# aleju/face-generator

Hardware: AMD Instinct MI355X
Metric: GAN train images/sec (G+D step) at 32x32x3 bs128 (higher is better)
Workload: dtype f32

## Files before the change

### face_generator_amd/csrc/thin.hip

```cpp
#include "fg_internal.h"
#ifdef FG_MEASURE
#define FG_THIN_DBG_BIT(v, b) ((v) & (b))
#else
#define FG_THIN_DBG_BIT(v, b) 0
#endif
#include <string.h>
#include <stdlib.h>
typedef float tw_f32x16 __attribute__((ext_vector_type(16)));
typedef float tw_f32x4 __attribute__((ext_vector_type(4)));

__device__ __forceinline__ float wave_sum_x(float v) {
#pragma unroll
    for (int o = 32; o > 0; o >>= 1) v += __shfl_xor(v, o, 64);
    return v;
}

template <int K, int CS, int CJ>
__global__ __launch_bounds__(256) void thin_in_kernel(const float* __restrict__ in, const float* __restrict__ Wp,
                                                      const float* __restrict__ bias, float* __restrict__ out, int B,
                                                      int H, int W, int flip, int Cw) {
    constexpr int PAD = (K - 1) / 2;
    const int lane = threadIdx.x & 63;
    const int wave = __builtin_amdgcn_readfirstlane(threadIdx.x >> 6);
    const int cb = blockIdx.y * (CJ * 64) + lane;
    float w[K * K * CS][CJ];
#pragma unroll
    for (int t = 0; t < K * K * CS; ++t)
#pragma unroll
        for (int j = 0; j < CJ; ++j) w[t][j] = Wp[(size_t)t * Cw + cb + 64 * j];
    float bv[CJ];
#pragma unroll
    for (int j = 0; j < CJ; ++j) bv[j] = bias ? bias[cb + 64 * j] : 0.f;
    const int npix = B * H * W;
    const int nwaves = gridDim.x * 4;
    for (int pix0 = blockIdx.x * 4 + wave; pix0 < npix; pix0 += 2 * nwaves) {
        float v[2][K * K * CS];
#pragma unroll
        for (int u = 0; u < 2; ++u) {
            const int pix = min(pix0 + u * nwaves, npix - 1);
            const int x = pix % W;
            const int t = pix / W;
            const int y = t % H;
            const int b = t / H;
#pragma unroll
            for (int dy = 0; dy < K; ++dy) {
                const int yy = y + (flip ? PAD - dy : dy - PAD);
                const int yc = min(max(yy, 0), H - 1);
#pragma unroll
                for (int dx = 0; dx < K; ++dx) {
                    const int xx = x + (flip ? PAD - dx : dx - PAD);
                    const int xc = min(max(xx, 0), W - 1);
                    const bool ok = yy == yc && xx == xc;
                    const float* ip = in + ((size_t)(b * H + yc) * W + xc) * CS;
#pragma unroll
                    for (int s = 0; s < CS; ++s) {
                        const float tv = ip[s];
                        v[u][(dy * K + dx) * CS + s] = ok ? tv : 0.f;
                    }
                }
            }
        }
#pragma unroll
        for (int u = 0; u < 2; ++u) {
            const int pix = pix0 + u * nwaves;
            if (pix >= npix) break;
            float acc[CJ];
#pragma unroll
            for (int j = 0; j < CJ; ++j) acc[j] = bv[j];
#pragma unroll
            for (int t = 0; t < K * K * CS; ++t)
#pragma unroll
                for (int j = 0; j < CJ; ++j) acc[j] = fmaf(v[u][t], w[t][j], acc[j]);
#pragma unroll
            for (int j = 0; j < CJ; ++j) out[(size_t)pix * Cw + cb + 64 * j] = acc[j];
        }
    }
}

template <int CS, int CJ>
__global__ __launch_bounds__(256) void thin_in_row3_kernel(const float* __restrict__ in, const float* __restrict__ Wp,
                                                           const float* __restrict__ bias, float* __restrict__ out,
                                                           int B, int H, int W, int flip, int Cw) {
    const int lane = threadIdx.x & 63;
    const int wave = __builtin_amdgcn_readfirstlane(threadIdx.x >> 6);
    const int cb = blockIdx.y * (CJ * 64) + lane;
    float w[9 * CS][CJ];
#pragma unroll
    for (int t = 0; t < 9; ++t)
#pragma unroll
        for (int s = 0; s < CS; ++s)
#pragma unroll
            for (int j = 0; j < CJ; ++j) w[t * CS + s][j] = Wp[(size_t)((flip ? 8 - t : t) * CS + s) * Cw + cb + 64 * j];
    float bv[CJ];
#pragma unroll
    for (int j = 0; j < CJ; ++j) bv[j] = bias ? bias[cb + 64 * j] : 0.f;
    const int row = blockIdx.x * 4 + wave;
    if (row >= B * H) return;
    const int y = row % H;
    const float* rp[3];
    bool rok[3];
#pragma unroll
    for (int dy = 0; dy < 3; ++dy) {
        const int yy = y + dy - 1;
        rok[dy] = (unsigned)yy < (unsigned)H;
        rp[dy] = in + (size_t)(row + (rok[dy] ? dy - 1 : 0)) * W * CS;
    }
    float win[3][3][CS];
#define FG_LOADCOL(slot, xc)                                                                        \
    {                                                                                               \
        const bool cok = (unsigned)(xc) < (unsigned)W;                                              \
        const int xcl = cok ? (xc) : 0;                                                             \
        _Pragma("unroll") for (int dy = 0; dy < 3; ++dy)                                            \
            _Pragma("unroll") for (int s = 0; s < CS; ++s) {                                        \
                const float tv = rp[dy][xcl * CS + s];                                              \
                win[slot][dy][s] = (cok && rok[dy]) ? tv : 0.f;                                     \
            }                                                                                       \
    }
    FG_LOADCOL(2, -1)
    FG_LOADCOL(0, 0)
    float* orow = out + (size_t)row * W * Cw + cb;
    for (int x0 = 0; x0 < W; x0 += 3) {
#pragma unroll
        for (int u = 0; u < 3; ++u) {
            const int x = x0 + u;
            if (x >= W) break;
            FG_LOADCOL((u + 1) % 3, x + 1)
            float acc[CJ];
#pragma unroll
            for (int j = 0; j < CJ; ++j) acc[j] = bv[j];
#pragma unroll
            for (int dy = 0; dy < 3; ++dy)
#pragma unroll
                for (int dx = 0; dx < 3; ++dx)
#pragma unroll
                    for (int s = 0; s < CS; ++s)
#pragma unroll
                        for (int j = 0; j < CJ; ++j)
                            acc[j] = fmaf(win[(u + dx + 2) % 3][dy][s], w[(dy * 3 + dx) * CS + s][j], acc[j]);
#pragma unroll
            for (int j = 0; j < CJ; ++j) orow[(size_t)x * Cw + 64 * j] = acc[j];
        }
    }
#undef FG_LOADCOL
}

template <int K, int CS>
__global__ __launch_bounds__(256) void thin_in_rows_kernel(const float* __restrict__ in, const float* __restrict__ Wp,
                                                           const float* __restrict__ bias, float* __restrict__ out,
                                                           int B, int H, int W, int flip, int Cw) {
    constexpr int PAD = (K - 1) / 2;
    constexpr int TR = 4, NPX = 4;
    constexpr int SEG = (NPX + K - 1) * CS;
    constexpr int SEG4 = (SEG + 3) / 4 * 4;
    extern __shared__ __attribute__((aligned(16))) float tile[];
    const int WP = (W + 2 * PAD + 3) / 4 * 4 + 4;
    const int lane = threadIdx.x & 63, wave = threadIdx.x >> 6;
    const int c = blockIdx.y * 64 + lane;
    float w[K * K * CS];
#pragma unroll
    for (int t = 0; t < K * K; ++t)
#pragma unroll
        for (int s = 0; s < CS; ++s) w[t * CS + s] = Wp[(size_t)((flip ? K * K - 1 - t : t) * CS + s) * Cw + c];
    const float bv = bias ? bias[c] : 0.f;
    const int strips_per_img = (H + TR - 1) / TR;
    const int b = blockIdx.x / strips_per_img, y0 = (blockIdx.x - b * strips_per_img) * TR;
    for (int i = threadIdx.x; i < (TR + 2 * PAD) * WP * CS; i += 256) {
        const int s = i % CS;
        const int t = i / CS;
        const int xx = t % WP - PAD, yy = y0 + t / WP - PAD;
        float v = 0.f;
        if ((unsigned)yy < (unsigned)H && (unsigned)xx < (unsigned)W) v = in[((size_t)(b * H + yy) * W + xx) * CS + s];
        tile[i] = v;
    }
    __syncthreads();
    const int rows = min(TR, H - y0);
    const int gpr = (W + NPX - 1) / NPX;
    for (int grp = wave; grp < rows * gpr; grp += 4) {
        const int r = grp / gpr, x0 = (grp - r * gpr) * NPX;
        float acc[NPX];
#pragma unroll
        for (int q = 0; q < NPX; ++q) acc[q] = bv;
#pragma unroll
        for (int dy = 0; dy < K; ++dy) {
            float seg[SEG4];
            const float* sp = tile + ((r + dy) * WP + x0) * CS;
#pragma unroll
            for (int i = 0; i < SEG4; ++i) seg[i] = sp[i];
#pragma unroll
            for (int dx = 0; dx < K; ++dx)
#pragma unroll
                for (int s = 0; s < CS; ++s)
#pragma unroll
                    for (int q = 0; q < NPX; ++q) acc[q] = fmaf(seg[(q + dx) * CS + s], w[(dy * K + dx) * CS + s], acc[q]);
            __builtin_amdgcn_sched_barrier(0);
        }
#pragma unroll
        for (int q = 0; q < NPX; ++q)
            if (x0 + q < W) out[((size_t)(b * H + y0 + r) * W + x0 + q) * Cw + c] = acc[q];
    }
}

__global__ __launch_bounds__(256) void thin_in_generic_kernel(const float* __restrict__ in, const float* __restrict__ Wp,
                                                              const float* __restrict__ bias, float* __restrict__ out,
                                                              int B, int H, int W, int Cs, int Cw, int K, int flip,
                                                              int cblk) {
    const int PAD = (K - 1) / 2;
    const int pl = threadIdx.x / cblk, tc = threadIdx.x - pl * cblk;
    const int PL = 256 / cblk;
    const int c = blockIdx.y * cblk + tc;
    const float bv = bias ? bias[c] : 0.f;
    const int npix = B * H * W;
    const int p0 = blockIdx.x * 128;
    for (int j = pl; j < 128; j += PL) {
        const int pix = p0 + j;
        if (pix >= npix) break;
        const int x = pix % W;
        const int t = pix / W;
        const int y = t % H;
        const int b = t / H;
        float acc = bv;
        for (int dy = 0; dy < K; ++dy) {
            const int yy = y + (flip ? PAD - dy : dy - PAD);
            if ((unsigned)yy >= (unsigned)H) continue;
            for (int dx = 0; dx < K; ++dx) {
                const int xx = x + (flip ? PAD - dx : dx - PAD);
                if ((unsigned)xx >= (unsigned)W) continue;
                const float* ip = in + ((size_t)(b * H + yy) * W + xx) * Cs;
                for (int s = 0; s < Cs; ++s) acc = fmaf(ip[s], Wp[(size_t)((dy * K + dx) * Cs + s) * Cw + c], acc);
            }
        }
        out[(size_t)pix * Cw + c] = acc;
    }
}

struct ThinEpi { const float* slope; float* y; const float* x; float* part; };
template <int EPI>
__device__ __forceinline__ void thin_epi_store(const ThinEpi& e, float sl, float* __restrict__ out, size_t idx, float v0, float v1,
                                               float x0, float x1, float& s) {
    if constexpr (EPI == 2) {
        s = fmaf(x0 > 0.f ? 0.f : x0, v0, s);
        s = fmaf(x1 > 0.f ? 0.f : x1, v1, s);
        out[idx] = x0 > 0.f ? v0 : sl * v0;
        out[idx + 32] = x1 > 0.f ? v1 : sl * v1;
    } else {
        out[idx] = v0;
        out[idx + 32] = v1;
        if constexpr (EPI == 1) {
            e.y[idx] = v0 > 0.f ? v0 : sl * v0;
            e.y[idx + 32] = v1 > 0.f ? v1 : sl * v1;
        }
    }
}
template <int EPI>
__device__ __forceinline__ void thin_epi_prefetch(const ThinEpi& e, int tile, int h, int npix, int Cw, int cbj, float (&x0)[16],
                                                  float (&x1)[16]) {
    if constexpr (EPI == 2) {
#pragma unroll
        for (int r = 0; r < 16; ++r) {
            const int p = tile * 32 + (r & 3) + 8 * (r >> 2) + 4 * h;
            const size_t idx = (size_t)(p < npix ? p : 0) * Cw + cbj;
            x0[r] = e.x[idx];
            x1[r] = e.x[idx + 32];
        }
    }
}
__device__ __forceinline__ void thin_epi_finish(const ThinEpi& e, float s, int lane, int wave) {
    if (!e.part) return;
#pragma unroll
    for (int o = 32; o > 0; o >>= 1) s += __shfl_xor(s, o, 64);
    if (lane == 0) e.part[((size_t)blockIdx.y * gridDim.x + blockIdx.x) * 4 + wave] = s;
}

template <int CS, int EPI>
__global__ __launch_bounds__(256) void thin_in_mfma_kernel(const float* __restrict__ in, const float* __restrict__ Wp,
                                                           const float* __restrict__ bias, float* __restrict__ out,
                                                           int npix, int H, int W, int flip, int Cw, int lgH, int lgW,
                                                           const ThinEpi epi, int nt_store) {
    constexpr int NA = 9 * CS;
    constexpr int KS = (NA + 1) / 2;
    constexpr int TS_LD = 68;
    __shared__ __attribute__((aligned(16))) float tsm[EPI == 0 ? 4 : 1][EPI == 0 ? 32 * TS_LD : 4];
    const int lane = threadIdx.x & 63, wave = threadIdx.x >> 6;
    const int cb = blockIdx.y * 64;
    const int h = lane >> 5, j = lane & 31;
    float wb[KS][2];
    int kdesc[KS];
#pragma unroll
    for (int ks = 0; ks < KS; ++ks) {
        const int k = 2 * ks + h;
        const bool valid = k < NA;
        const int tap = valid ? k / CS : 0, sc = valid ? k - tap * CS : 0;
        const size_t widx = (size_t)((flip ? 8 - tap : tap) * CS + sc) * Cw + cb + j;
        wb[ks][0] = valid ? Wp[widx] : 0.f;
        wb[ks][1] = valid ? Wp[widx + 32] : 0.f;
        kdesc[ks] = (tap / 3) | ((tap % 3) << 2) | (sc << 4) | ((valid ? 1 : 0) << 8);
    }
    const float b0 = bias ? bias[cb + j] : 0.f, b1 = bias ? bias[cb + 32 + j] : 0.f;
    const bool p2 = lgW >= 0 && lgH >= 0;
    const int ntiles = (npix + 31) / 32;
    const float esl = EPI ? epi.slope[0] : 1.f;
    float es = 0.f;
    auto load_a = [&](int tile, float (&av)[KS]) {
        const int pix = tile * 32 + j;
        const bool ok = pix < npix;
        int x, y, t;
        if (p2) { x = pix & (W - 1); t = pix >> lgW; y = t & (H - 1); }
        else { t = pix / W; x = pix - t * W; y = t % H; }
#pragma unroll
        for (int ks = 0; ks < KS; ++ks) {
            const int d = kdesc[ks];
            const int yy = y + (d & 3) - 1, xx = x + ((d >> 2) & 3) - 1;
            float a = 0.f;
// ... 841 lines not shown
            }                                                                                                        \
            hipLaunchKernelGGL((thin_out_rows_mfma_kernel<KK, CC>), grid, dim3(256), lds, ctx->stream, in, Wp, rbuf, B, H, W, Cw); \
            FG_CHECK_LAUNCH(ctx);                                                                                    \
            hipLaunchKernelGGL((thin_out_rows_gather_kernel<KK, CC>), dim3(fg_cdiv(npix * CC, 256)), dim3(256), 0,    \
                               ctx->stream, rbuf, bias, out, npix, W, sigmoid);                                      \
            FG_CHECK_LAUNCH(ctx);                                                                                    \
            return FG_OK;                                                                                            \
        }
        TOR(5, 1) TOR(5, 3) TOR(7, 1) TOR(7, 3)
#undef TOR
    }
    dim3 grid(fg_cdiv(npix, 64));
    const long long in_bytes = (long long)npix * Cw * 4;
    {
        const bool use_slab = (ctx->fusion & FG_FUSE_THIN_SLAB) != 0;
        int R = 0;
        if (W >= 4 && W <= 128) {
            const int rmax = (80 * 1024 / (29 * 4)) / W - 2;
            int rt = (int)(((long long)H * B + 255) / 256);
            if (rt > rmax) rt = rmax;
            if (rt > H) rt = H;
            if (rt < 2) rt = 2;
            for (int pass = 0; pass < 2 && !R; ++pass)
                for (int r = rt; r >= 2; --r)
                    if (((r + 2) * W) % 32 == 0 && (pass == 1 || H % r == 0)) { R = r; break; }
            if (!R && rmax >= 2)
                for (int r = rt + 1; r <= rmax; ++r) if (((r + 2) * W) % 32 == 0) { R = r; break; }
        }
        if (use_slab && in_bytes < (long long)FG_OOB_T && k == 3 && R >= 2 && (Cw == 64 || Cw == 128) && Cs <= 3 &&
            ((R + 2) * W) % 32 == 0) {
            const int nblk = B * ((H + R - 1) / R);
            const size_t lds = (size_t)(R + 2) * W * 29 * sizeof(float);
#define TOS(JJ, CC)                                                                                                  \
            if (Cw == JJ * 64 && Cs == CC) {                                                                         \
                static bool attr = false;                                                                            \
                if (!attr) {                                                                                         \
                    FG_HIP(ctx, hipFuncSetAttribute((const void*)thin_out_slab_mfma_kernel<JJ, CC>,                  \
                                                    hipFuncAttributeMaxDynamicSharedMemorySize, 160 * 1024));        \
                    attr = true;                                                                                     \
                }                                                                                                    \
                hipLaunchKernelGGL((thin_out_slab_mfma_kernel<JJ, CC>), dim3(nblk), dim3(256), lds, ctx->stream, in, Wp, bias, \
                                   out, H, W, R, flip, sigmoid, (int)in_bytes);                                      \
                FG_CHECK_LAUNCH(ctx);                                                                                \
                return FG_OK;                                                                                        \
            }
            TOS(1, 1) TOS(1, 3) TOS(2, 1) TOS(2, 3)
#undef TOS
        }
    }
    if (in_bytes < (long long)FG_OOB_T && k == 3 && W % 4 == 0) {
        int nblk = fg_cdiv(fg_cdiv(npix, 4), 4);
        if (nblk > 4096) nblk = 4096;
#define TOW(JJ, CC)                                                                                                  \
        if (Cw == JJ * 64 && Cs == CC) {                                                                             \
            hipLaunchKernelGGL((thin_out_win_kernel<JJ, CC>), dim3(nblk), dim3(256), 0, ctx->stream, in, Wp, bias, out, B, H, \
                               W, flip, sigmoid, (int)in_bytes);                                                     \
            FG_CHECK_LAUNCH(ctx);                                                                                    \
            return FG_OK;                                                                                            \
        }
        TOW(1, 1) TOW(1, 3) TOW(2, 1) TOW(2, 3)
#undef TOW
    }
    if (in_bytes < (long long)FG_OOB_T) {
        int nblk = fg_cdiv(fg_cdiv(npix, 4), 4);
        if (nblk > 4096) nblk = 4096;
#define TO(KK, JJ, CC)                                                                                              \
    if (k == KK && Cw == JJ * 64 && Cs == CC) {                                                                     \
        hipLaunchKernelGGL((thin_out_kernel<KK, JJ, CC, 4>), dim3(nblk), dim3(256), 0, ctx->stream, in, Wp, bias, out, B, \
                           H, W, flip, sigmoid, (int)in_bytes);                                                     \
        FG_CHECK_LAUNCH(ctx);                                                                                       \
        return FG_OK;                                                                                               \
    }
        TO(3, 1, 1) TO(3, 1, 3) TO(3, 2, 1) TO(3, 2, 3)
    }
#undef TO
    if (Cw % 32 == 0 && (k == 3 || k == 5 || k == 7) && (Cs == 1 || Cs == 3)) {
        const int tp = 16 + k - 1;
        const size_t lds = (size_t)tp * tp * 36 * sizeof(float);
        dim3 tgrid(B * ((H + 15) / 16) * ((W + 15) / 16));
#define TOT(KK, CC)                                                                                                  \
    if (k == KK && Cs == CC) {                                                                                       \
        static bool attr = false;                                                                                    \
        if (!attr) {                                                                                                 \
            FG_HIP(ctx, hipFuncSetAttribute((const void*)thin_out_tiled_kernel<KK, CC>,                              \
                                            hipFuncAttributeMaxDynamicSharedMemorySize, (int)lds));                  \
            attr = true;                                                                                             \
        }                                                                                                            \
        hipLaunchKernelGGL((thin_out_tiled_kernel<KK, CC>), tgrid, dim3(256), lds, ctx->stream, in, Wp, bias, out, B, H, \
                           W, Cw, flip, sigmoid);                                                                    \
        FG_CHECK_LAUNCH(ctx);                                                                                        \
        return FG_OK;                                                                                                \
    }
        TOT(3, 1) TOT(3, 3) TOT(5, 1) TOT(5, 3) TOT(7, 1) TOT(7, 3)
#undef TOT
    }
    hipLaunchKernelGGL(thin_out_generic_kernel, grid, dim3(256), 0, ctx->stream, in, Wp, bias, out, B, H, W, Cw, Cs, k,
                       flip, sigmoid);
    FG_CHECK_LAUNCH(ctx);
    return FG_OK;
}

#define TW_BLOCKS FG_THIN_WGRAD_BLOCKS
#define TW_ROWS 4
template <int K, int CS>
__global__ __launch_bounds__(256) void thin_wgrad_kernel(const float* __restrict__ thin, const float* __restrict__ wide,
                                                         float* __restrict__ part, int B, int H, int W, int Cw, int sgn,
                                                         int cblk) {
    constexpr int PAD = (K - 1) / 2;
    constexpr int NA = K * K * CS;
    extern __shared__ float sh[];
    const int WP = W + 2 * PAD;
    float* tile = sh;
    float* red = sh + (TW_ROWS + 2 * PAD) * WP * CS;
    const int pl = threadIdx.x / cblk, tc = threadIdx.x - pl * cblk;
    const int PL = 256 / cblk;
    const int c = blockIdx.y * cblk + tc;
    const int strips_per_img = (H + TW_ROWS - 1) / TW_ROWS;
    const int nstrips = B * strips_per_img;
    float acc[NA];
#pragma unroll
    for (int t = 0; t < NA; ++t) acc[t] = 0.f;
    for (int st = blockIdx.x; st < nstrips; st += gridDim.x) {
        const int b = st / strips_per_img, y0 = (st - b * strips_per_img) * TW_ROWS;
        __syncthreads();
        for (int i = threadIdx.x; i < (TW_ROWS + 2 * PAD) * WP * CS; i += 256) {
            const int s = i % CS;
            const int t = i / CS;
            const int xx = t % WP - PAD, yy = y0 + t / WP - PAD;
            float v = 0.f;
            if ((unsigned)yy < (unsigned)H && (unsigned)xx < (unsigned)W) v = thin[((size_t)(b * H + yy) * W + xx) * CS + s];
            tile[i] = v;
        }
        __syncthreads();
        const int rows = min(TW_ROWS, H - y0);
        const int npx = rows * W;
        for (int j0 = pl; j0 < npx; j0 += 4 * PL) {
            float wv[4];
#pragma unroll
            for (int u = 0; u < 4; ++u) {
                const int j = j0 + u * PL;
                wv[u] = j < npx ? wide[((size_t)(b * H + y0) * W + j) * Cw + c] : 0.f;
            }
#pragma unroll
            for (int u = 0; u < 4; ++u) {
                const int j = j0 + u * PL;
                if (j >= npx) break;
                const int ry = j / W, rx = j - ry * W;
#pragma unroll
                for (int dy = 0; dy < K; ++dy)
#pragma unroll
                    for (int dx = 0; dx < K; ++dx) {
                        const float* tp = tile + ((ry + PAD + sgn * (dy - PAD)) * WP + rx + PAD + sgn * (dx - PAD)) * CS;
#pragma unroll
                        for (int s = 0; s < CS; ++s)
                            acc[(dy * K + dx) * CS + s] = fmaf(tp[s], wv[u], acc[(dy * K + dx) * CS + s]);
                    }
            }
        }
    }
    float* dst = part + (size_t)blockIdx.x * NA * Cw;
    if (PL == 1) {
#pragma unroll
        for (int t = 0; t < NA; ++t) dst[(size_t)t * Cw + c] = acc[t];
    } else {
        __syncthreads();
#pragma unroll
        for (int t = 0; t < NA; ++t) red[(pl * NA + t) * cblk + tc] = acc[t];
        __syncthreads();
        if (pl == 0) {
#pragma unroll
            for (int t = 0; t < NA; ++t) {
                float s = 0.f;
                for (int q = 0; q < PL; ++q) s += red[(q * NA + t) * cblk + tc];
                dst[(size_t)t * Cw + c] = s;
            }
        }
    }
}

template <int K, int CS, int PADDED = 0, int ONES = 0>
__global__ __launch_bounds__(256) void thin_wgrad_mfma_kernel(const float* __restrict__ thin, const float* __restrict__ wide,
                                                              float* __restrict__ part, int B, int H, int W, int Cw, int sgn, int lgH, int lgW) {
    constexpr int PAD = (K - 1) / 2;
    constexpr int NA = K * K * CS;
    constexpr int NCT = (NA + 31) / 32;
    static_assert(NA % 32 != 0, "the ones column needs an idle column");
    constexpr int CTO = NA / 32;
    __shared__ float red[4][2][16][64];
    const int lane = threadIdx.x & 63, wave = threadIdx.x >> 6;
    const int cbase = blockIdx.y * 64;
    const long long npix = (long long)B * H * W, npairs = (npix + 1) / 2;
    const int j = lane & 31, k = lane >> 5;
    const bool ones_lane = ONES && (CTO * 32 + j == NA);
    constexpr int NR = NA + ONES;
    int oy[NCT], ox[NCT], sch[NCT];
    bool jok[NCT];
#pragma unroll
    for (int ct = 0; ct < NCT; ++ct) {
        const int jj = ct * 32 + j;
        jok[ct] = jj < NA;
        const int tap = jok[ct] ? jj / CS : 0;
        sch[ct] = jok[ct] ? jj - tap * CS : 0;
        oy[ct] = sgn * (tap / K - PAD); ox[ct] = sgn * (tap % K - PAD);
    }
    const int Wp = W + 2 * PAD;
    int poff[NCT];
#pragma unroll
    for (int ct = 0; ct < NCT; ++ct) poff[ct] = (oy[ct] * Wp + ox[ct]) * CS + sch[ct];
    tw_f32x16 acc[NCT][2];
#pragma unroll
    for (int ct = 0; ct < NCT; ++ct)
#pragma unroll
        for (int r = 0; r < 16; ++r) { acc[ct][0][r] = 0.f; acc[ct][1][r] = 0.f; }
    const int npx = (int)npix, npr = (int)npairs;
    const int stride = gridDim.x * 4;
    const bool p2 = lgW >= 0 && lgH >= 0;
    constexpr int U = NCT <= 2 ? 2 : 1;
    if constexpr (PADDED) {
        constexpr int TW_OOB = 0x7FFFFFF0;
        const __amdgpu_buffer_rsrc_t wrs = __builtin_amdgcn_make_buffer_rsrc((void*)wide, 0, npx * Cw * 4, 0x00020000);
        const __amdgpu_buffer_rsrc_t trs = __builtin_amdgcn_make_buffer_rsrc((void*)thin, 0, B * (H + 2 * PAD) * Wp * CS * 4, 0x00020000);
        const int wlane = (cbase + j) * 4, wrow = Cw * 4;
        int poffB[NCT];
#pragma unroll
        for (int ct = 0; ct < NCT; ++ct) poffB[ct] = poff[ct] * 4;
        auto fetch = [&](int pp, float& a0, float& a1, float (&bv)[NCT]) {
            const int pix = 2 * pp + k;
            const bool ok = pp < npr && pix < npx;
            const int wo = ok ? pix * wrow + wlane : TW_OOB;
            a0 = __uint_as_float(__builtin_amdgcn_raw_buffer_load_b32(wrs, wo, 0, 0));
            a1 = __uint_as_float(__builtin_amdgcn_raw_buffer_load_b32(wrs, wo + 128, 0, 0));
            const int pc = ok ? pix : 0;
            const int x = pc & (W - 1), row = pc >> lgW, b = row >> lgH;
            const int base = (((row + b * (2 * PAD) + PAD) * Wp + x + PAD) * CS) * 4;
#pragma unroll
            for (int ct = 0; ct < NCT; ++ct) bv[ct] = __uint_as_float(__builtin_amdgcn_raw_buffer_load_b32(trs, base + poffB[ct], 0, 0));
            if constexpr (ONES) { if (ones_lane) bv[CTO] = 1.f; }
        };
        auto mul = [&](float a0, float a1, const float (&bv)[NCT]) {
#pragma unroll
            for (int ct = 0; ct < NCT; ++ct) {
                acc[ct][0] = __builtin_amdgcn_mfma_f32_32x32x2f32(a0, bv[ct], acc[ct][0], 0, 0, 0);
                acc[ct][1] = __builtin_amdgcn_mfma_f32_32x32x2f32(a1, bv[ct], acc[ct][1], 0, 0, 0);
            }
        };
        float a0A, a1A, bA[NCT], a0B, a1B, bB[NCT];
        int pp = blockIdx.x * 4 + wave;
        fetch(pp, a0A, a1A, bA);
        for (; pp < npr; pp += 2 * stride) {
            fetch(pp + stride, a0B, a1B, bB);
            __builtin_amdgcn_sched_barrier(0);
            mul(a0A, a1A, bA);
            __builtin_amdgcn_sched_barrier(0);
            fetch(pp + 2 * stride, a0A, a1A, bA);
            __builtin_amdgcn_sched_barrier(0);
            mul(a0B, a1B, bB);
            __builtin_amdgcn_sched_barrier(0);
        }
    } else
    for (int pp0 = blockIdx.x * 4 + wave; pp0 < npr; pp0 += U * stride) {
        float a0[U], a1[U], bv[U][NCT];
#pragma unroll
        for (int u = 0; u < U; ++u) {
            const int pp = pp0 + u * stride;
            const int pix = 2 * pp + k;
            a0[u] = 0.f; a1[u] = 0.f;
#pragma unroll
            for (int ct = 0; ct < NCT; ++ct) bv[u][ct] = 0.f;
            if (pp < npr && pix < npx) {
                const float* wp = wide + (size_t)pix * Cw + cbase + j;
                a0[u] = wp[0]; a1[u] = wp[32];
                int x, y, t;
                if (p2) { x = pix & (W - 1); t = pix >> lgW; y = t & (H - 1); }
                else { t = pix / W; x = pix - t * W; y = t % H; }
#pragma unroll
                for (int ct = 0; ct < NCT; ++ct) {
                    const int yy = y + oy[ct], xx = x + ox[ct];
                    if (jok[ct] && (unsigned)yy < (unsigned)H && (unsigned)xx < (unsigned)W)
                        bv[u][ct] = thin[(size_t)((t - y + yy) * W + xx) * CS + sch[ct]];
                }
                if constexpr (ONES) { if (ones_lane) bv[u][CTO] = 1.f; }
            }
        }
#pragma unroll
        for (int u = 0; u < U; ++u)
#pragma unroll
            for (int ct = 0; ct < NCT; ++ct) {
                acc[ct][0] = __builtin_amdgcn_mfma_f32_32x32x2f32(a0[u], bv[u][ct], acc[ct][0], 0, 0, 0);
                acc[ct][1] = __builtin_amdgcn_mfma_f32_32x32x2f32(a1[u], bv[u][ct], acc[ct][1], 0, 0, 0);
            }
    }
    float* dst = part + (size_t)blockIdx.x * NR * Cw;
#pragma unroll
    for (int ct = 0; ct < NCT; ++ct) {
        if (ct) __syncthreads();
#pragma unroll
        for (int r = 0; r < 16; ++r) { red[wave][0][r][lane] = acc[ct][0][r]; red[wave][1][r][lane] = acc[ct][1][r]; }
        __syncthreads();
        for (int e = threadIdx.x; e < 2 * 16 * 64; e += 256) {
            const int tile = e >> 10, r = (e >> 6) & 15, l = e & 63;
            const int col = ct * 32 + (l & 31), row = (r & 3) + 8 * (r >> 2) + 4 * (l >> 5);
            if (col < NR)
                dst[(size_t)col * Cw + cbase + tile * 32 + row] = (red[0][tile][r][l] + red[1][tile][r][l]) + (red[2][tile][r][l] + red[3][tile][r][l]);
        }
    }
}

int fg_launch_thin_wgrad(fg_ctx* ctx, const float* thin, const float* wide, float* gw_tsc, int B, int H, int W, int Cs,
                         int Cw, int k, int shift_thin, float* scratch, float* wide_colsum, int* colsum_done, float* gradW_ref,
                         int unpack_mode, int* unpacked) {
    if (colsum_done) *colsum_done = 0;
    if (unpacked) *unpacked = 0;
    if (Cw % 64) return fg_set_err(ctx, FG_ERR_INVALID, "thin_wgrad: Cw %% 64");
    const int ones = (wide_colsum && colsum_done && k == 3 && (ctx->fusion & FG_FUSE_THIN_BIAS)) ? 1 : 0;
    const int NR = k * k * Cs + ones;
    auto finish = [&](int nblocks) -> int {
        if (gradW_ref && unpacked) {
            *unpacked = 1;
            if (ones) *colsum_done = 1;
            const int O = unpack_mode == 0 ? Cw : Cs, I = unpack_mode == 0 ? Cs : Cw;
            return fg_launch_colsum_final_thin(ctx, scratch, nblocks, gradW_ref, O, I, k, unpack_mode, ones ? Cw : 0, wide_colsum);
        }
        if (!ones) return fg_launch_colsum_final(ctx, scratch, nblocks, NR * Cw, 0.f, gw_tsc);
        *colsum_done = 1;
        return fg_launch_colsum_final2(ctx, scratch, nblocks, (NR - 1) * Cw, gw_tsc, Cw, wide_colsum);
    };
    char plabel[48] = "";
    if (ctx->prof) snprintf(plabel, sizeof(plabel), "thin_wgrad<%d,%d>", k, Cs);
    FgProfScope prof(ctx, fg_intern(ctx, plabel), 2.0 * B * H * W * (double)k * k * Cs * Cw, 0.0, 4.0 * B * H * W * ((double)Cw + Cs));
    {
        const long long npairs = ((long long)B * H * W + 1) / 2;
        int nb = (int)((npairs + 3) / 4 < TW_BLOCKS ? (npairs + 3) / 4 : TW_BLOCKS);
        if (nb < 1) nb = 1;
        dim3 grid(nb, Cw / 64);
        int lgH = -1, lgW = -1;
        for (int q = 0; q < 15; ++q) { if ((1 << q) == H) lgH = q; if ((1 << q) == W) lgW = q; }
        const bool fits = (long long)B * H * W * Cw < (1LL << 31);
        if (fits && k >= 5 && lgH >= 0 && lgW >= 0 && (Cs == 1 || Cs == 3)) {
            const int pad = (k - 1) / 2;
            const long long slab = (long long)NR * Cw, padf = (long long)B * (H + 2 * pad) * (W + 2 * pad) * Cs;
            const long long take = (padf + slab - 1) / slab;
            if (take <= TW_BLOCKS / 4 && padf < (1LL << 28) && (long long)B * H * W * Cw * 4 < 0x7FFFFFF0LL) {
                const int nbp = nb < TW_BLOCKS - (int)take ? nb : TW_BLOCKS - (int)take;
                float* padded = scratch + (long long)(TW_BLOCKS - take) * slab;
{ const int rcp = fg_launch_thin_pad(ctx, thin, padded, B, H, W, Cs, pad); if (rcp) return rcp; }
                dim3 gridp(nbp, Cw / 64);
#define TWP(KK, CC)                                                                                                  \
                if (k == KK && Cs == CC) {                                                                           \
                    hipLaunchKernelGGL((thin_wgrad_mfma_kernel<KK, CC, 1>), gridp, dim3(256), 0, ctx->stream, padded, wide, scratch, B, \
                                       H, W, Cw, shift_thin, lgH, lgW);                                              \
                    FG_CHECK_LAUNCH(ctx);                                                                            \
                    return finish(nbp);                                                                              \
                }
                TWP(5, 1) TWP(5, 3) TWP(7, 1) TWP(7, 3)
#undef TWP
            }
        }
#define TWM(KK, CC)                                                                                                  \
        if (fits && k == KK && Cs == CC) {                                                                           \
            if (KK == 3 && ones)                                                                                     \
                hipLaunchKernelGGL((thin_wgrad_mfma_kernel<KK, CC, 0, (KK == 3 ? 1 : 0)>), grid, dim3(256), 0, ctx->stream, thin, wide, \
                                   scratch, B, H, W, Cw, shift_thin, lgH, lgW);                                      \
            else                                                                                                     \
                hipLaunchKernelGGL((thin_wgrad_mfma_kernel<KK, CC>), grid, dim3(256), 0, ctx->stream, thin, wide, scratch, B, H, \
                                   W, Cw, shift_thin, lgH, lgW);                                                     \
            FG_CHECK_LAUNCH(ctx);                                                                                    \
            return finish(nb);                                                                                       \
        }
        TWM(3, 1) TWM(3, 3) TWM(3, 4) TWM(5, 1) TWM(5, 3) TWM(7, 1) TWM(7, 3)
#undef TWM
    }
    const int cblk = Cw >= 256 ? 256 : Cw;
    if (Cw % cblk || 256 % cblk) return fg_set_err(ctx, FG_ERR_INVALID, "thin_wgrad: Cw=%d unsupported", Cw);
    const int nstrips = B * ((H + TW_ROWS - 1) / TW_ROWS);
    int nb = nstrips < TW_BLOCKS ? nstrips : TW_BLOCKS;
    if (nb < 1) nb = 1;
    const int PL = 256 / cblk;
    const int NA = k * k * Cs;
    const int pad = (k - 1) / 2;
    dim3 grid(nb, Cw / cblk);
    const size_t lds = ((size_t)(TW_ROWS + 2 * pad) * (W + 2 * pad) * Cs + (PL > 1 ? (size_t)PL * NA * cblk : 0)) * sizeof(float);
#define TWG(KK, CC)                                                                                                  \
    if (k == KK && Cs == CC) {                                                                                       \
        hipLaunchKernelGGL((thin_wgrad_kernel<KK, CC>), grid, dim3(256), lds, ctx->stream, thin, wide, scratch, B, H, W, \
                           Cw, shift_thin, cblk);                                                                    \
        FG_CHECK_LAUNCH(ctx);                                                                                        \
        return fg_launch_colsum_final(ctx, scratch, nb, NA * Cw, 0.f, gw_tsc);                                       \
    }
    TWG(3, 1) TWG(3, 3) TWG(3, 4) TWG(5, 3) TWG(7, 3) TWG(7, 1)
#undef TWG
    return fg_set_err(ctx, FG_ERR_UNSUPPORTED, "thin_wgrad: k=%d Cs=%d not built", k, Cs);
}

__global__ void thin_pack_kernel(const float* __restrict__ Wr, float* __restrict__ Wp, int O, int I, int kk, int mode) {
    const int total = O * I * kk;
    const int idx = blockIdx.x * blockDim.x + threadIdx.x;
    if (idx >= total) return;
    const int Cs = mode == 0 ? I : O, Cw = mode == 0 ? O : I;
    const int c = idx % Cw;
    const int t = idx / Cw;
    const int s = t % Cs;
    const int tap = t / Cs;
    const int o = mode == 0 ? c : s, i = mode == 0 ? s : c;
    Wp[idx] = Wr[((size_t)o * I + i) * kk + tap];
}
int fg_launch_thin_pack(fg_ctx* ctx, const float* W, float* Wp, int O, int I, int k, int mode) {
    const int total = O * I * k * k;
    hipLaunchKernelGGL(thin_pack_kernel, dim3(fg_cdiv(total, 256)), dim3(256), 0, ctx->stream, W, Wp, O, I, k * k, mode);
    FG_CHECK_LAUNCH(ctx);
    return FG_OK;
}
__global__ void thin_unpack_grad_kernel(const float* __restrict__ gw, float* __restrict__ gradW, int O, int I, int kk,
                                        int mode, float beta) {
    const int total = O * I * kk;
    const int idx = blockIdx.x * blockDim.x + threadIdx.x;
    if (idx >= total) return;
    const int Cs = mode == 0 ? I : O, Cw = mode == 0 ? O : I;
    const int c = idx % Cw;
    const int t = idx / Cw;
    const int s = t % Cs;
    const int tap = t / Cs;
    const int o = mode == 0 ? c : s, i = mode == 0 ? s : c;
    const size_t r = ((size_t)o * I + i) * kk + tap;
    gradW[r] = (beta == 0.f ? 0.f : beta * gradW[r]) + gw[idx];
}
int fg_launch_thin_unpack_grad(fg_ctx* ctx, const float* gw, float* gradW, int O, int I, int k, int mode, float beta) {
    const int total = O * I * k * k;
    hipLaunchKernelGGL(thin_unpack_grad_kernel, dim3(fg_cdiv(total, 256)), dim3(256), 0, ctx->stream, gw, gradW, O, I,
                       k * k, mode, beta);
    FG_CHECK_LAUNCH(ctx);
    return FG_OK;
}
```

Baseline: 49400.

## Add streaming double-buffered MFMA weight-gradient kernel for 3x3 thin convs

Adds a new 3x3 thin-channel weight-gradient kernel that walks pixel pairs across the grid. It loads wide activations with 64-bit buffer loads and uses buffer-load bounds handling in place of explicit padding. Fetches and MFMA accumulation are double-buffered and split by sched barriers so memory latency overlaps the matrix work. The 3x3 path now routes to this kernel ahead of the existing mfma kernel, which adds register pressure and a new reduction index mapping that could be wrong.

```diff
diff --git a/face_generator_amd/csrc/thin.hip b/face_generator_amd/csrc/thin.hip
--- a/face_generator_amd/csrc/thin.hip
+++ b/face_generator_amd/csrc/thin.hip
@@ -8,6 +8,7 @@
 #include <stdlib.h>
 typedef float tw_f32x16 __attribute__((ext_vector_type(16)));
 typedef float tw_f32x4 __attribute__((ext_vector_type(4)));
+typedef float tw_f32x2 __attribute__((ext_vector_type(2)));
 
 __device__ __forceinline__ float wave_sum_x(float v) {
 #pragma unroll
@@ -1455,6 +1456,107 @@
             const int col = ct * 32 + (l & 31), row = (r & 3) + 8 * (r >> 2) + 4 * (l >> 5);
             if (col < NR)
                 dst[(size_t)col * Cw + cbase + tile * 32 + row] = (red[0][tile][r][l] + red[1][tile][r][l]) + (red[2][tile][r][l] + red[3][tile][r][l]);
+        }
+    }
+}
+
+template <int CS, int ONES>
+__global__ __launch_bounds__(256) void thin_wgrad3_stream_kernel(const float* __restrict__ thin, const float* __restrict__ wide,
+                                                                 float* __restrict__ part, int B, int H, int W, int Cw, int sgn, int lgH, int lgW) {
+    constexpr int V = 2;
+    constexpr int NA = 9 * CS;
+    constexpr int NCT = (NA + 31) / 32;
+    static_assert(NA % 32 != 0, "the ones column needs an idle column");
+    constexpr int CTO = NA / 32;
+    constexpr int NR = NA + ONES;
+    constexpr int U = 4;
+    constexpr int TW_OOB = 0x7FFFFFF0;
+    constexpr int RLD = 65;
+    __shared__ float red[4][2][16][RLD];
+    const int lane = threadIdx.x & 63, wave = threadIdx.x >> 6;
+    const int cbase = blockIdx.y * (32 * V);
+    const int j = lane & 31, k = lane >> 5;
+    const int npx = B * H * W, npr = (npx + 1) / 2;
+    const bool ones_lane = ONES && (CTO * 32 + j == NA);
+    int oy[NCT], ox[NCT], doff[NCT];
+    bool jok[NCT];
+#pragma unroll
+    for (int ct = 0; ct < NCT; ++ct) {
+        const int jj = ct * 32 + j;
+        jok[ct] = jj < NA;
+        const int tap = jok[ct] ? jj / CS : 0;
+        const int sch = jok[ct] ? jj - tap * CS : 0;
+        oy[ct] = sgn * (tap / 3 - 1); ox[ct] = sgn * (tap % 3 - 1);
+        doff[ct] = ((oy[ct] * W + ox[ct]) * CS + sch) * 4;
+    }
+    tw_f32x16 acc[NCT][V];
+#pragma unroll
+    for (int ct = 0; ct < NCT; ++ct)
+#pragma unroll
+        for (int v = 0; v < V; ++v)
+#pragma unroll
+            for (int r = 0; r < 16; ++r) acc[ct][v][r] = 0.f;
+    const __amdgpu_buffer_rsrc_t wrs = __builtin_amdgcn_make_buffer_rsrc((void*)wide, 0, npx * Cw * 4, 0x00020000);
+    const __amdgpu_buffer_rsrc_t trs = __builtin_amdgcn_make_buffer_rsrc((void*)thin, 0, npx * CS * 4, 0x00020000);
+    const int wlane = (cbase + V * j) * 4, wrow = Cw * 4;
+    const bool p2 = lgW >= 0 && lgH >= 0;
+    const int stride = gridDim.x * 4;
+    auto fetch = [&](int pp0, float (&a)[U][V], float (&bv)[U][NCT]) {
+#pragma unroll
+        for (int u = 0; u < U; ++u) {
+            const int pp = pp0 + u * stride;
+            const int pix = 2 * pp + k;
+            const bool ok = pp < npr && pix < npx;
+            const int pc = ok ? pix : 0;
+            const int wo = ok ? pc * wrow + wlane : TW_OOB;
+            const tw_f32x2 t2 = __builtin_bit_cast(tw_f32x2, __builtin_amdgcn_raw_buffer_load_b64(wrs, wo, 0, 0));
+            a[u][0] = t2[0]; a[u][1] = t2[1];
+            int x, y;
+            if (p2) { x = pc & (W - 1); y = (pc >> lgW) & (H - 1); }
+            else { const int t = pc / W; x = pc - t * W; y = t % H; }
+            const int tbase = pc * (CS * 4);
+#pragma unroll
+            for (int ct = 0; ct < NCT; ++ct) {
+                const bool in = ok && jok[ct] && (unsigned)(y + oy[ct]) < (unsigned)H && (unsigned)(x + ox[ct]) < (unsigned)W;
+                bv[u][ct] = __uint_as_float(__builtin_amdgcn_raw_buffer_load_b32(trs, in ? tbase + doff[ct] : TW_OOB, 0, 0));
+            }
+            if constexpr (ONES) { if (ones_lane) bv[u][CTO] = 1.f; }
+        }
+    };
+    auto mul = [&](const float (&a)[U][V], const float (&bv)[U][NCT]) {
+#pragma unroll
+        for (int u = 0; u < U; ++u)
+#pragma unroll
+            for (int ct = 0; ct < NCT; ++ct)
+#pragma unroll
+                for (int v = 0; v < V; ++v) acc[ct][v] = __builtin_amdgcn_mfma_f32_32x32x2f32(a[u][v], bv[u][ct], acc[ct][v], 0, 0, 0);
+    };
+    float aA[U][V], bA[U][NCT], aB[U][V], bB[U][NCT];
+    int pp = blockIdx.x * 4 + wave;
+    fetch(pp, aA, bA);
+    for (; pp < npr; pp += 2 * U * stride) {
+        fetch(pp + U * stride, aB, bB);
+        __builtin_amdgcn_sched_barrier(0);
+        mul(aA, bA);
+        __builtin_amdgcn_sched_barrier(0);
+        fetch(pp + 2 * U * stride, aA, bA);
+        __builtin_amdgcn_sched_barrier(0);
+        mul(aB, bB);
+        __builtin_amdgcn_sched_barrier(0);
+    }
+    float* dst = part + (size_t)blockIdx.x * NR * Cw;
+#pragma unroll
+    for (int ct = 0; ct < NCT; ++ct) {
+        if (ct) __syncthreads();
+#pragma unroll
+        for (int r = 0; r < 16; ++r) { red[wave][0][r][lane] = acc[ct][0][r]; red[wave][1][r][lane] = acc[ct][1][r]; }
+        __syncthreads();
+        for (int e = threadIdx.x; e < 32 * 64; e += 256) {
+            const int ch = e & 63, col = ct * 32 + (e >> 6);
+            const int tile = ch & 1, row = ch >> 1;
+            const int r = (row & 3) | ((row >> 3) << 2), l = (e >> 6) + 8 * (row & 4);
+            if (col < NR)
+                dst[(size_t)col * Cw + cbase + ch] = (red[0][tile][r][l] + red[1][tile][r][l]) + (red[2][tile][r][l] + red[3][tile][r][l]);
         }
     }
 }
@@ -1509,8 +1611,24 @@
 #undef TWP
             }
         }
+        if (k == 3 && (long long)B * H * W * Cw * 4 < 0x7FFFFFF0LL) {
+            dim3 grids(nb, Cw / 64);
+#define TWS(CC)                                                                                                      \
+            if (Cs == CC) {                                                                                          \
+                if (ones)                                                                                            \
+                    hipLaunchKernelGGL((thin_wgrad3_stream_kernel<CC, 1>), grids, dim3(256), 0, ctx->stream, thin, wide, scratch, B, H, \
+                                       W, Cw, shift_thin, lgH, lgW);                                                 \
+                else                                                                                                 \
+                    hipLaunchKernelGGL((thin_wgrad3_stream_kernel<CC, 0>), grids, dim3(256), 0, ctx->stream, thin, wide, scratch, B, H, \
+                                       W, Cw, shift_thin, lgH, lgW);                                                 \
+                FG_CHECK_LAUNCH(ctx);                                                                                \
+                return finish(nb);                                                                                   \
+            }
+            TWS(1) TWS(3) TWS(4)
+#undef TWS
+        }
 #define TWM(KK, CC)                                                                                                  \
-        if (fits && k == KK && Cs == CC) {                                                                           \
+        if (fits && k == KK && Cs == CC) {                                                                        \
             if (KK == 3 && ones)                                                                                     \
                 hipLaunchKernelGGL((thin_wgrad_mfma_kernel<KK, CC, 0, (KK == 3 ? 1 : 0)>), grid, dim3(256), 0, ctx->stream, thin, wide, \
                                    scratch, B, H, W, Cw, shift_thin, lgH, lgW);                                      \
```

Result: no change. 49660 (median of 6 runs) (+0.5%).
